# AlgoLab/rs-vgaligner

Measured on AMD Instinct MI355X. Metric: aligned reads/sec (10 kbp ONT vs HLA graph), higher is better.
Workload: dtype int32+f64

## Files before the change

### rs-vgaligner_amd/csrc/vga_poa_row.hpp

```cpp
#pragma once

#include "vga_poa_launch.hpp"
#include "vga_poa_kernels.hpp"

#define T4_NEG (4 * POA_NEG)

template <int B>
__device__ __forceinline__ int t4_sub_byte(int a, int g)
{
    int r;
    if constexpr (B == 0) asm("v_sub_u32_sdwa %0, %1, %2 dst_sel:DWORD dst_unused:UNUSED_PAD src0_sel:DWORD src1_sel:BYTE_0" : "=v"(r) : "v"(a), "v"(g));
    if constexpr (B == 1) asm("v_sub_u32_sdwa %0, %1, %2 dst_sel:DWORD dst_unused:UNUSED_PAD src0_sel:DWORD src1_sel:BYTE_1" : "=v"(r) : "v"(a), "v"(g));
    if constexpr (B == 2) asm("v_sub_u32_sdwa %0, %1, %2 dst_sel:DWORD dst_unused:UNUSED_PAD src0_sel:DWORD src1_sel:BYTE_2" : "=v"(r) : "v"(a), "v"(g));
    if constexpr (B == 3) asm("v_sub_u32_sdwa %0, %1, %2 dst_sel:DWORD dst_unused:UNUSED_PAD src0_sel:DWORD src1_sel:BYTE_3" : "=v"(r) : "v"(a), "v"(g));
    return r;
}
template <int B>
__device__ __forceinline__ void t4_gap_byte(int &dst, int &acc, int t, int c)
{
    if constexpr (B == 0) asm("v_min_u32_sdwa %0, %2, %3 dst_sel:BYTE_0 dst_unused:UNUSED_PRESERVE src0_sel:DWORD src1_sel:DWORD\n\tv_cmp_le_u32 vcc, %3, %2\n\tv_addc_co_u32 %1, vcc, %1, %1, vcc" : "+v"(dst), "+v"(acc) : "v"(t), "s"(c) : "vcc");
    if constexpr (B == 1) asm("v_min_u32_sdwa %0, %2, %3 dst_sel:BYTE_1 dst_unused:UNUSED_PRESERVE src0_sel:DWORD src1_sel:DWORD\n\tv_cmp_le_u32 vcc, %3, %2\n\tv_addc_co_u32 %1, vcc, %1, %1, vcc" : "+v"(dst), "+v"(acc) : "v"(t), "s"(c) : "vcc");
    if constexpr (B == 2) asm("v_min_u32_sdwa %0, %2, %3 dst_sel:BYTE_2 dst_unused:UNUSED_PRESERVE src0_sel:DWORD src1_sel:DWORD\n\tv_cmp_le_u32 vcc, %3, %2\n\tv_addc_co_u32 %1, vcc, %1, %1, vcc" : "+v"(dst), "+v"(acc) : "v"(t), "s"(c) : "vcc");
    if constexpr (B == 3) asm("v_min_u32_sdwa %0, %2, %3 dst_sel:BYTE_3 dst_unused:UNUSED_PRESERVE src0_sel:DWORD src1_sel:DWORD\n\tv_cmp_le_u32 vcc, %3, %2\n\tv_addc_co_u32 %1, vcc, %1, %1, vcc" : "+v"(dst), "+v"(acc) : "v"(t), "s"(c) : "vcc");
}
__device__ __forceinline__ void t4_flag_ne(int &acc, int a, int b)
{
    asm("v_cmp_ne_u32 vcc, %1, %2\n\tv_addc_co_u32 %0, vcc, %0, %0, vcc" : "+v"(acc) : "v"(a), "v"(b) : "vcc");
}
template <int B>
__device__ __forceinline__ void t4_flag_ne_dep(int &dst, int acc, int a, int b)
{
    if constexpr (B == 0) asm("v_cmp_ne_u32 vcc, %2, %3\n\tv_addc_co_u32_sdwa %0, vcc, %1, %1, vcc dst_sel:BYTE_0 dst_unused:UNUSED_PRESERVE src0_sel:DWORD src1_sel:DWORD" : "+v"(dst) : "v"(acc), "v"(a), "v"(b) : "vcc");
    if constexpr (B == 1) asm("v_cmp_ne_u32 vcc, %2, %3\n\tv_addc_co_u32_sdwa %0, vcc, %1, %1, vcc dst_sel:BYTE_1 dst_unused:UNUSED_PRESERVE src0_sel:DWORD src1_sel:DWORD" : "+v"(dst) : "v"(acc), "v"(a), "v"(b) : "vcc");
    if constexpr (B == 2) asm("v_cmp_ne_u32 vcc, %2, %3\n\tv_addc_co_u32_sdwa %0, vcc, %1, %1, vcc dst_sel:BYTE_2 dst_unused:UNUSED_PRESERVE src0_sel:DWORD src1_sel:DWORD" : "+v"(dst) : "v"(acc), "v"(a), "v"(b) : "vcc");
    if constexpr (B == 3) asm("v_cmp_ne_u32 vcc, %2, %3\n\tv_addc_co_u32_sdwa %0, vcc, %1, %1, vcc dst_sel:BYTE_3 dst_unused:UNUSED_PRESERVE src0_sel:DWORD src1_sel:DWORD" : "+v"(dst) : "v"(acc), "v"(a), "v"(b) : "vcc");
}
__device__ __forceinline__ int t4_max3(int a, int b, int c)
{
    int r;
    asm("v_max3_i32 %0, %1, %2, %3" : "=v"(r) : "v"(a), "v"(b), "v"(c));
    return r;
}
__device__ __forceinline__ int t4_shr1_max(int v, int pre)
{
    int r = pre;
    asm("s_nop 1\n\tv_max_i32_dpp %0, %1, %2 wave_shr:1 row_mask:0xf bank_mask:0xf" : "+v"(r) : "v"(v), "v"(pre));
    return r;
}
__device__ __forceinline__ int t4_shr1_mov(int v, int first)
{
    int r = first;
    asm("s_nop 1\n\tv_mov_b32_dpp %0, %1 wave_shr:1 row_mask:0xf bank_mask:0xf" : "+v"(r) : "v"(v));
    return r;
}

template <int B>
__device__ __forceinline__ void t5_min_byte(int &dst, int t, int c)
{
    if constexpr (B == 0) asm("v_min_u32_sdwa %0, %1, %2 dst_sel:BYTE_0 dst_unused:UNUSED_PRESERVE src0_sel:DWORD src1_sel:DWORD" : "+v"(dst) : "v"(t), "s"(c));
    if constexpr (B == 1) asm("v_min_u32_sdwa %0, %1, %2 dst_sel:BYTE_1 dst_unused:UNUSED_PRESERVE src0_sel:DWORD src1_sel:DWORD" : "+v"(dst) : "v"(t), "s"(c));
    if constexpr (B == 2) asm("v_min_u32_sdwa %0, %1, %2 dst_sel:BYTE_2 dst_unused:UNUSED_PRESERVE src0_sel:DWORD src1_sel:DWORD" : "+v"(dst) : "v"(t), "s"(c));
    if constexpr (B == 3) asm("v_min_u32_sdwa %0, %1, %2 dst_sel:BYTE_3 dst_unused:UNUSED_PRESERVE src0_sel:DWORD src1_sel:DWORD" : "+v"(dst) : "v"(t), "s"(c));
}

__device__ __forceinline__ int t5_own(int v)
{
    asm volatile("" : "+v"(v));
    return __builtin_amdgcn_readfirstlane(v);
}
__device__ __forceinline__ uint32_t t5_own(uint32_t v) { return (uint32_t)t5_own((int)v); }
__device__ __forceinline__ uint64_t t5_own(uint64_t v) { return ((uint64_t)t5_own((uint32_t)(v >> 32)) << 32) | t5_own((uint32_t)v); }
template <typename T>
__device__ __forceinline__ T *t5_own(T *p) { return (T *)t5_own((uint64_t)p); }


struct poa_row_view {
    int qlen;
    const char *query;
    const uint4 *ntab;
    const uint32_t *plist, *seqw;
    poa_row *R;
    uint32_t n_nodes, ring_rows;
    int bw, banded, p_match, p_mismatch;
};
__device__ __forceinline__ poa_row_view poa_row_view_of(const poa_prob &pb, const char *queries, const uint4 *node_tab, const uint32_t *seq32,
                                                        const uint32_t *preds, const poa_t5_args &A)
{
    poa_row_view V;
    V.qlen = t5_own((int)pb.qlen);
    V.query = queries + pb.q0;
    V.ntab = node_tab + t5_own(pb.node0);
    V.plist = preds + t5_own(pb.pred0);
    V.seqw = seq32 + t5_own(pb.seq0 >> 2);
    V.R = A.rows + t5_own(pb.row0);
    V.n_nodes = t5_own(pb.n_nodes);
    V.ring_rows = t5_own(pb.ring_rows);
    V.bw = t5_own((int)pb.w);
    V.banded = t5_own(A.P.banded);
    V.p_match = t5_own(A.P.match);
    V.p_mismatch = t5_own(A.P.mismatch);
    return V;
}
struct poa_row_pen {
    int o1, e1, o2, e2, D1, D2;
    uint32_t g_bias, e_probe;
};
template <bool DEF>
__device__ __forceinline__ poa_row_pen poa_row_pen_of(const poa_dev_params &P)
{
    poa_row_pen K;
    K.o1 = DEF ? 4 : t5_own(P.o1); K.e1 = DEF ? 2 : t5_own(P.e1); K.o2 = DEF ? 24 : t5_own(P.o2); K.e2 = DEF ? 1 : t5_own(P.e2);
    K.D1 = 4 * K.o1; K.D2 = 4 * K.o2 + 1;
    K.g_bias = (uint32_t)(4 * K.e1 | (4 * K.e2) << 8) * 0x00010001u;
    K.e_probe = (uint32_t)((128 - K.D1) | (128 - K.D2) << 8) * 0x00010001u;
    return K;
}

__device__ __forceinline__ bool poa_row_state(const poa_t5_args &A, int got, bool first_thread, uint64_t &state_lo)
{
    if (got < 0) {
        if (first_thread) {
            poa_out &O = A.outs[blockIdx.x];
            O.t_end = O.t_begin; O.cells = 0; O.vcells = 0; O.maxw = 0; O.nops = 0;
            O.score = POA_NEG; O.row = 0; O.status = A.cp.n_slots ? POA_ST_POOL : POA_ST_RETRY;
        }
        return false;
    }
    __builtin_amdgcn_fence(__ATOMIC_ACQUIRE, "agent");
    state_lo = (uint64_t)A.cp.state_base + (uint64_t)(uint32_t)got * A.cp.state_size;
    return true;
}

struct poa_chunks {
    uint32_t own_head, own_tail, own_chunks;
    uint64_t dcur;
    uint32_t drem;
};
__device__ __forceinline__ uint32_t poa_chunks_pop(const poa_chunk_pool &cp, const poa_chunks &C)
{
    const uint32_t idx = poa_chunk_pop(cp, blockIdx.x);
    if (idx != POA_NIL) __hip_atomic_store(cp.next + idx, C.own_head, __ATOMIC_RELAXED, __HIP_MEMORY_SCOPE_AGENT);
    return idx;
}
__device__ __forceinline__ void poa_chunks_took(poa_chunks &C, uint32_t idx, uint64_t addr)
{
    C.own_head = idx;
    if (C.own_tail == POA_NIL) C.own_tail = idx;
    C.own_chunks++;
    C.dcur = addr;
    C.drem = (uint32_t)POA_CHUNK;
}
__device__ __forceinline__ uint64_t poa_chunks_bump(poa_chunks &C, uint32_t bytes)
{
    const uint64_t r = C.dcur;
    C.dcur += bytes;
    C.drem -= bytes;
    return r;
}

__device__ __forceinline__ int poa_row_codes(uint16_t *Qn, const char *query, int qlen, int n_hw, int tid, int nt)
{
    int non_acgt = 0;
    for (int t = tid; t < n_hw; t += nt) {
        uint32_t hw = 0;
#pragma unroll
        for (int k = 0; k < 4; k++) {
            const int j = 4 * t + k;
            uint32_t code = 0;
            if (j >= 1 && j <= qlen) {
                const char ch = query[j - 1];
                code = (ch == 'A' || ch == 'C' || ch == 'G' || ch == 'T') ? 1u << (((uint32_t)ch >> 1) & 3u) : 0u;
                non_acgt |= code == 0;
            }
            hw |= code << (4 * k);
        }
        Qn[t] = (uint16_t)hw;
    }
    return non_acgt;
}

struct poa_row_topo {
    uint32_t r;
    bool last;
    bool is_sink;
    uint32_t ps;
    uint32_t gb;
    bool simple;
    bool first;
    int np;
    int remain;
};
__device__ __forceinline__ poa_row_topo poa_row_topo_of(const uint4 nt, uint32_t v, uint32_t tn, const uint32_t *seqw, uint32_t &seq_word,
                                                        uint32_t &seq_word_idx)
{
    const uint32_t nlen = nt.y & 0xFFFFFFu;
    const int np_node = (int)(nt.y >> 24);
    poa_row_topo T;
    T.r = nt.x + tn;
    T.last = tn + 1 == nlen;
    T.is_sink = T.last && (nt.z >> 31) != 0;
    T.ps = nt.w;
    T.gb = 0;
    if (v > 0) {
        const uint32_t bi = T.r - 1;
        if ((bi & 3u) == 0 || (bi >> 2) != seq_word_idx) { seq_word_idx = bi >> 2; seq_word = seqw[seq_word_idx]; }
        T.gb = (seq_word >> (8u * (bi & 3u))) & 0xffu;
    }
    T.simple = T.r > 0 && (tn > 0 || (np_node == 1 && T.ps == T.r - 1));
    T.first = tn == 0 && v > 0;
    T.np = v == 0 ? 0 : (tn == 0 ? np_node : 1);
    T.remain = (int)(nt.z & 0x3fffffffu) + (int)(nlen - 1 - tn);
    return T;
}

__device__ __forceinline__ void poa_row_far_span(const poa_row_view &V, const poa_row_topo &T, int prev_lmax, int prev_rmax, int &mpl, int &mpr)
{
    mpl = INT32_MAX; mpr = 0;
    for (int t = 0; t < T.np; t++) {
        const uint32_t p = T.np == 1 ? T.ps : V.plist[T.ps + t];
        int lm, rm;
        if (p == T.r - 1) { lm = prev_lmax + 1; rm = prev_rmax + 1; }
        else {
            lm = __builtin_amdgcn_readfirstlane(V.R[p].lmax) + 1;
            rm = __builtin_amdgcn_readfirstlane(V.R[p].rmax) + 1;
        }
        mpl = lm < mpl ? lm : mpl;
        mpr = rm > mpr ? rm : mpr;
    }
}
__device__ __forceinline__ void poa_row_band(const poa_row_view &V, const poa_row_topo &T, int mpl, int mpr, int &beg, int &end, int &bal, int &W)
{
    if (!V.banded) { beg = 0; end = V.qlen; }
    else {
        const int diag = V.qlen - T.remain;
        const int lo = mpl < diag ? mpl : diag;
        const int hi = mpr > diag ? mpr : diag;
        beg = lo - V.bw; if (beg < 0) beg = 0;
        end = hi + V.bw; if (end > V.qlen) end = V.qlen;
    }
    bal = beg & ~3;
    W = (end - bal + 1 + 3) & ~3;
}

__device__ __forceinline__ uint32_t poa_row_dir_bytes(int W, int np) { return (uint32_t)W * (np > 1 ? 4u : 1u); }
__device__ __forceinline__ bool poa_row_value_in_chunk(const poa_row_topo &T, const uint4 nt) { return T.r == 0 || (nt.z & 0x40000000u); }
__device__ __forceinline__ uint64_t poa_row_ring_slot(uint64_t ring_base, uint32_t ring_size, uint32_t ring_rows, uint32_t &ring_head)
{
    const uint64_t voff = ring_base + (uint64_t)ring_head * ring_size;
    ring_head = ring_head + 1 == ring_rows ? 0 : ring_head + 1;
    return voff;
}
struct poa_row_counts {
    uint64_t cells, vcells;
    int maxw;
};
__device__ __forceinline__ void poa_row_record(poa_row *R, const poa_row_topo &T, bool first_thread, int beg, int end, int W, uint64_t doff,
                                               uint64_t voff, poa_row_counts &N)
{
    if (T.r > 0) N.cells += (uint64_t)(end - beg + 1);
    if (T.last) N.vcells += (uint64_t)(end - beg + 1);
    N.maxw = W > N.maxw ? W : N.maxw;
    if (first_thread) {
        *(int4 *)&R[T.r].beg = make_int4(beg, end, (int)(uint32_t)doff, (int)(uint32_t)(doff >> 32));
        *(uint2 *)&R[T.r].pred = make_uint2(T.ps, T.first ? (uint32_t)T.np : 0u);
        if (T.last) R[T.r].voff = voff;
    }
}

struct poa_row_base {
    int gsh, ne4t, mm4;
};
__device__ __forceinline__ poa_row_base poa_row_base_of(uint32_t gb, int p_match, int p_mismatch)
{
    const uint32_t gd = gb - (uint32_t)'A';
    const bool acgt = gd < 20u && ((0x80045u >> gd) & 1u);
    const int sc_eq = acgt ? p_match : 0, sc_ne = acgt ? -p_mismatch : 0;
    poa_row_base B;
    B.gsh = (int)((gb >> 1) & 3u);
    B.ne4t = 4 * sc_ne + 1;
    B.mm4 = 4 * (sc_eq - sc_ne);
    return B;
}

struct poa_pred_row {
    const uint8_t *Vq;
    int bp, balq, Wq;
    unsigned pspan;
};
__device__ __forceinline__ poa_pred_row poa_pred_row_of(const poa_row *R, uint32_t p)
{
    poa_pred_row P;
    P.bp = __builtin_amdgcn_readfirstlane(R[p].beg);
    const int ep = __builtin_amdgcn_readfirstlane(R[p].end);
    const uint64_t vq_off = poa_uniform_u64(R[p].voff);
    P.Vq = (const uint8_t *)vq_off;
    P.balq = P.bp & ~3;
    P.Wq = vq_off != 0 ? (ep - P.balq + 1 + 3) & ~3 : 0;
    P.pspan = (unsigned)(ep - P.bp);
    return P;
}
__device__ __forceinline__ void poa_pred_quad(const poa_pred_row &P, int j0, int fill, int4 &hv, uint2 &gg)
{
    const int idx = j0 - P.balq;
    hv = make_int4(fill, fill, fill, fill);
    gg = make_uint2(0u, 0u);
    if (idx >= 0 && idx < P.Wq) {
        hv = *(const int4 *)((const int32_t *)P.Vq + idx);
        gg = *(const uint2 *)(P.Vq + 4ll * P.Wq + 2ll * idx);
    }
}
__device__ __forceinline__ int poa_pred_word(const poa_pred_row &P, int j, int fill)
{
    const int idx = j - P.balq;
    return (idx >= 0 && idx < P.Wq) ? ((const int32_t *)P.Vq)[idx] : fill;
}
__device__ __forceinline__ void poa_stage_quad(const poa_pred_row &P, int j0, int4 &hv, uint2 &gg)
{
    poa_pred_quad(P, j0, T4_NEG + 1, hv, gg);
    const unsigned pspan = P.pspan;
    const bool in0 = (unsigned)(j0 - P.bp) <= pspan, in1 = (unsigned)(j0 + 1 - P.bp) <= pspan, in2 = (unsigned)(j0 + 2 - P.bp) <= pspan,
               in3 = (unsigned)(j0 + 3 - P.bp) <= pspan;
    hv.x = in0 ? hv.x : T4_NEG + 1; hv.y = in1 ? hv.y : T4_NEG + 1; hv.z = in2 ? hv.z : T4_NEG + 1; hv.w = in3 ? hv.w : T4_NEG + 1;
    gg.x = (in0 ? gg.x & 0xffffu : 0u) | (in1 ? gg.x & 0xffff0000u : 0u);
    gg.y = (in2 ? gg.y & 0xffffu : 0u) | (in3 ? gg.y & 0xffff0000u : 0u);
}
__device__ __forceinline__ int poa_stage_word(const poa_pred_row &P, int j)
{
    const int wl = poa_pred_word(P, j, T4_NEG + 1);
    return (unsigned)(j - P.bp) <= P.pspan ? wl : T4_NEG + 1;
}
template <int Q>
struct poa_merged {
    int h[Q][4];
    uint32_t ga[Q], gb[Q];
    int hl;
    bool no_row;
};
template <int Q>
__device__ __forceinline__ poa_merged<Q> poa_stage_merge(const poa_row_view &V, const poa_row_topo &T, int jl, int bal, int W, uint8_t *drow)
{
    poa_merged<Q> M;
    int x1[Q][4], x2[Q][4];
    uint32_t ah[Q], a1[Q], a2[Q];
    uint32_t ahl = 0;
    M.no_row = false;
    M.hl = T4_NEG;
#pragma unroll
    for (int q = 0; q < Q; q++) {
        ah[q] = 0; a1[q] = 0; a2[q] = 0;
#pragma unroll
        for (int k = 0; k < 4; k++) { M.h[q][k] = T4_NEG; x1[q][k] = T4_NEG; x2[q][k] = T4_NEG; }
    }
    for (int t = 0; t < T.np; t++) {
        const poa_pred_row P = poa_pred_row_of(V.R, V.plist[T.ps + t]);
        if (__builtin_expect(P.Vq == nullptr, 0)) M.no_row = true;
#pragma unroll
        for (int q = 0; q < Q; q++) {
            const int j0 = jl + 4 * q;
            int4 hv;
            uint2 gg;
            poa_pred_quad(P, j0, 0, hv, gg);
            const int hj[4] = {hv.x, hv.y, hv.z, hv.w};
            const uint32_t g16[4] = {gg.x & 0xffffu, gg.x >> 16, gg.y & 0xffffu, gg.y >> 16};
#pragma unroll
            for (int k = 0; k < 4; k++) {
// ... 145 lines not shown
```

### rs-vgaligner_amd/csrc/vga_poa_t5.hpp

```cpp
#pragma once

#include "vga_poa_row.hpp"

__device__ __forceinline__ uint64_t t5_uniform64(uint64_t v)
{
    return ((uint64_t)(uint32_t)__builtin_amdgcn_readfirstlane((int)(v >> 32)) << 32) | (uint32_t)__builtin_amdgcn_readfirstlane((int)(uint32_t)v);
}

#define POA_T5_ARGS_OFFSET 40
__device__ __forceinline__ const poa_t5_args *t5_kargs()
{
    uint32_t off = POA_T5_ARGS_OFFSET;
    asm volatile("" : "+s"(off));
    return (const poa_t5_args *)((const char *)__builtin_amdgcn_kernarg_segment_ptr() + off);
}
template <int NT, bool DEF>
__global__ __launch_bounds__(NT) __attribute__((amdgpu_waves_per_eu(5)))
void k_poa_dp_t5(const poa_prob *__restrict__ probs, const char *__restrict__ queries,
                                                       const uint4 *__restrict__ node_tab, const uint32_t *__restrict__ seq32,
                                                       const uint32_t *__restrict__ preds, const poa_t5_args A)
{
    poa_row *rows = A.rows;
    uint8_t *pool_arg = A.pool;
    const uint32_t lds_cols = t5_own(A.lds_cols), hg_cols = t5_own(A.hg_cols), win_mask = t5_own(A.win_mask);
    enum : uint32_t { ST_CHUNKED = 1u, ST_QPLAIN = 2u, ST_FAILED = 4u, ST_PREV_LDS = 8u, ST_PREV_FAR_USE = 16u };
    uint32_t st = (A.cp.n_slots != 0 ? ST_CHUNKED : 0u) | ST_PREV_LDS;
#define chunked ((st & ST_CHUNKED) != 0)
#define failed ((st & ST_FAILED) != 0)
#define q_plain ((st & ST_QPLAIN) != 0)
#define prev_lds ((st & ST_PREV_LDS) != 0)
#define prev_far_use ((st & ST_PREV_FAR_USE) != 0)
    struct { int match, mismatch, o1, e1, o2, e2, banded; } P = {t5_own(A.P.match), t5_own(A.P.mismatch), A.P.o1, A.P.e1, A.P.o2, A.P.e2, t5_own(A.P.banded)};
    constexpr int NW = NT / 64;
    constexpr int STEP = NT * 4;
    extern __shared__ __attribute__((aligned(16))) uint8_t smem[];
    int4 *sX = (int4 *)smem;
    int4 *sRed = sX + 2 * NW;
    int32_t *edgeW = (int32_t *)(sRed + NW);
    int32_t *sSink = edgeW + 4;
    uint64_t *sChunk = (uint64_t *)(sSink + 4);
    constexpr int HDR = (3 * NW + 1 + 1 + 2) * 16;
    int32_t *Hs = (int32_t *)(smem + HDR);
    uint16_t *Gs = (uint16_t *)(smem + HDR + 4ull * hg_cols);
    uint16_t *Qn = (uint16_t *)(smem + HDR + 6ull * hg_cols);
    const int edge_idx = (int)(edgeW - Hs);

    if (threadIdx.x == 0) A.outs[blockIdx.x].t_begin = __builtin_amdgcn_s_memrealtime();
    if (A.prio) __builtin_amdgcn_s_setprio(3);
    const poa_prob pb = probs[blockIdx.x];
    const int tid = threadIdx.x, lane = tid & 63, wv = __builtin_amdgcn_readfirstlane(tid >> 6);
    const int qlen = t5_own((int)pb.qlen);
    const char *query = queries + pb.q0;
    const uint4 *ntab = node_tab + t5_own(pb.node0);
    const uint32_t *plist = preds + t5_own(pb.pred0);
    const uint32_t *seqw = seq32 + t5_own(pb.seq0 >> 2);
    poa_row *R = rows + t5_own(pb.row0);
    const uint32_t n_nodes = t5_own(pb.n_nodes), ring_rows = t5_own(pb.ring_rows);

    uint8_t *pool = pool_arg;
    uint64_t state_lo = 0, state_hi = 0;
    if (chunked) {
        int got = -1;
        if (!(pb.flags & 1u)) {
            if (tid == 0) {
                got = poa_slot_acquire(A.cp.slot_flag, A.cp.n_slots, blockIdx.x);
                sSink[1] = got;
            }
            __syncthreads();
            got = __builtin_amdgcn_readfirstlane(sSink[1]);
        }
        if (got < 0) {
            if (tid == 0) {
                poa_out &O = A.outs[blockIdx.x];
                O.t_end = O.t_begin; O.cells = 0; O.vcells = 0; O.maxw = 0; O.nops = 0;
                O.score = POA_NEG; O.row = 0; O.status = POA_ST_POOL;
            }
            return;
        }
        __builtin_amdgcn_fence(__ATOMIC_ACQUIRE, "agent");
        pool = nullptr;
        state_lo = (uint64_t)A.cp.state_base + (uint64_t)(uint32_t)got * A.cp.state_size;
        state_hi = state_lo + A.cp.state_size;
    }

    const int o1 = DEF ? 4 : P.o1, e1 = DEF ? 2 : P.e1, o2 = DEF ? 24 : P.o2, e2 = DEF ? 1 : P.e2;
    const int C1 = 4 * (o1 + e1), C2 = 4 * (o2 + e2) + 1;
    const int D1 = 4 * o1, D2 = 4 * o2 + 1;
    const uint32_t g_bias = (uint32_t)(4 * e1 | (4 * e2) << 8) * 0x00010001u;
    const uint32_t e_probe = (uint32_t)((128 - D1) | (128 - D2) << 8) * 0x00010001u;
    const int bw = t5_own((int)pb.w);

    uint32_t own_head = POA_NIL, own_chunks = 0;
    auto alloc = [&](uint64_t &cur, uint32_t &rem, uint32_t bytes_asked, int slot) -> uint64_t {
        const uint32_t bytes = (bytes_asked + 15u) & ~15u;
        if (__builtin_expect(bytes > rem, 0)) {
            if (chunked) {
                if (slot == 0 && bytes <= POA_CHUNK) {
                    const poa_t5_args *ka = t5_kargs();
                    if (tid == 0) {
                        const uint32_t idx = poa_chunk_pop(ka->cp, blockIdx.x);
                        if (idx != POA_NIL) __hip_atomic_store(ka->cp.next + idx, own_head, __ATOMIC_RELAXED, __HIP_MEMORY_SCOPE_AGENT);
                        if (own_chunks == 0) sChunk[3] = idx;
                        sChunk[0] = idx;
                    }
                    __syncthreads();
                    const uint32_t idx = (uint32_t)__builtin_amdgcn_readfirstlane((int)(uint32_t)sChunk[0]);
                    __syncthreads();
                    if (idx == POA_NIL) st |= ST_FAILED;
                    else {
                        own_head = idx;
                        own_chunks++;
                        cur = poa_uniform_u64(poa_chunk_addr(ka->cp, idx));
                        rem = (uint32_t)POA_CHUNK;
                    }
                } else
                    st |= ST_FAILED;
                if (failed) return cur;
            } else {
                const uint64_t need = bytes > POA_CHUNK ? ((uint64_t)bytes + POA_CHUNK - 1) & ~(POA_CHUNK - 1) : POA_CHUNK;
                const poa_t5_args *ka = t5_kargs();
                if (tid == 0) sChunk[slot] = atomicAdd(ka->pool_next, (unsigned long long)need);
                __syncthreads();
                const uint64_t b = t5_uniform64(sChunk[slot]);
                __syncthreads();
                if (b + need > ka->pool_size) st |= ST_FAILED;
                cur = b;
                rem = (uint32_t)need;
            }
        }
        const uint64_t r = cur;
        cur += bytes;
        rem -= bytes;
        return r;
    };

    int non_acgt = 0;
    for (int t = tid; t < (int)(lds_cols / 4); t += NT) {
        uint32_t hw = 0;
#pragma unroll
        for (int k = 0; k < 4; k++) {
            const int j = 4 * t + k;
            uint32_t code = 0;
            if (j >= 1 && j <= qlen) {
                const char ch = query[j - 1];
                code = (ch == 'A' || ch == 'C' || ch == 'G' || ch == 'T') ? 1u << (((uint32_t)ch >> 1) & 3u) : 0u;
                non_acgt |= code == 0;
            }
            hw |= code << (4 * k);
        }
        Qn[t] = (uint16_t)hw;
    }
    if (__builtin_amdgcn_readfirstlane(__syncthreads_or(non_acgt)) == 0) st |= ST_QPLAIN;

    uint64_t dcur = 0, vcur = state_lo, wide_scratch = 0, ring_base = 0;
    uint32_t dend = 0, vendp = (uint32_t)(state_hi - state_lo);
    uint32_t ring_head = 0;
    if (win_mask != 0xFFFFFFFFu) wide_scratch = alloc(vcur, vendp, 2u * 6u * lds_cols, 1);
    {
        const uint64_t maxrow = (6ull * (uint64_t)((qlen + 8) & ~3) + 15ull) & ~15ull;
        if (chunked) {
            ring_base = alloc(vcur, vendp, (uint32_t)(maxrow * (uint64_t)ring_rows), 1);
        } else {
            const uint64_t rb = (maxrow * (uint64_t)ring_rows + POA_CHUNK - 1) & ~(POA_CHUNK - 1);
            if (tid == 0) sChunk[2] = atomicAdd(A.pool_next, (unsigned long long)rb);
            __syncthreads();
            const uint64_t b = t5_uniform64(sChunk[2]);
            if (b + rb > A.pool_size || rb >= (1ull << 32)) st |= ST_FAILED;
            ring_base = b;
        }
    }
    if (tid == 0) { sSink[2] = POA_NEG; sSink[3] = 0; }
    int prev_beg = 0, prev_end = -1;
    uint32_t seq_word = 0, seq_word_idx = 0xFFFFFFFFu;

    for (uint32_t v = 0; v < n_nodes && !failed; v++) {
    const uint4 nt = ntab[v];
    const uint32_t nlen = nt.y & 0xFFFFFFu;
    for (uint32_t tn = 0; tn < nlen && !failed; tn++) {
        asm volatile("" : "+s"(st));
        POA_MARK("row_topo");
        const uint32_t r = nt.x + tn;
        const bool last = tn + 1 == nlen;
        const bool is_sink = last && (nt.z >> 31) != 0;
        const uint32_t ps = nt.w;
        uint32_t gb = 0;
        if (v > 0) {
            const uint32_t bi = r - 1;
            if ((bi & 3u) == 0 || (bi >> 2) != seq_word_idx) { seq_word_idx = bi >> 2; seq_word = seqw[seq_word_idx]; }
            gb = (seq_word >> (8u * (bi & 3u))) & 0xffu;
        }
        const bool simple = r > 0 && prev_lds && (tn > 0 || ((nt.y >> 24) == 1u && ps == r - 1));
        const bool writer = wv == (int)(r % (uint32_t)NW);
        POA_MARK("row_prevmax");
        int prev_lmax = 0, prev_rmax = 0;
        if (r > 0) {
            int4 rw = make_int4(INT32_MIN, INT32_MAX, INT32_MIN, 0);
            if (lane < NW) rw = sRed[lane];
            int b = rw.x, t;
            t = poa_dpp<0x111, 0xf>(INT32_MIN, b); b = t > b ? t : b;
            if (NW > 2) { t = poa_dpp<0x112, 0xf>(INT32_MIN, b); b = t > b ? t : b; }
            if (NW > 4) { t = poa_dpp<0x114, 0xf>(INT32_MIN, b); b = t > b ? t : b; }
            if (NW > 8) { t = poa_dpp<0x118, 0xf>(INT32_MIN, b); b = t > b ? t : b; }
            const int rbest = __builtin_amdgcn_readlane(b, NW - 1);
            const uint64_t tie = __builtin_amdgcn_ballot_w64(rw.x == rbest);
            if (__builtin_expect(__builtin_popcountll(tie) == 1, 1)) {
                const int w1 = __builtin_ctzll(tie);
                prev_lmax = __builtin_amdgcn_readlane(rw.y, w1);
                prev_rmax = __builtin_amdgcn_readlane(rw.z, w1);
            } else {
                int lm = rw.x == rbest ? rw.y : INT32_MAX, rm = rw.x == rbest ? rw.z : INT32_MIN;
                t = poa_dpp<0x111, 0xf>(INT32_MAX, lm); lm = t < lm ? t : lm;
                t = poa_dpp<0x111, 0xf>(INT32_MIN, rm); rm = t > rm ? t : rm;
                if (NW > 2) {
                    t = poa_dpp<0x112, 0xf>(INT32_MAX, lm); lm = t < lm ? t : lm;
                    t = poa_dpp<0x112, 0xf>(INT32_MIN, rm); rm = t > rm ? t : rm;
                }
                if (NW > 4) {
                    t = poa_dpp<0x114, 0xf>(INT32_MAX, lm); lm = t < lm ? t : lm;
                    t = poa_dpp<0x114, 0xf>(INT32_MIN, rm); rm = t > rm ? t : rm;
                }
                if (NW > 8) {
                    t = poa_dpp<0x118, 0xf>(INT32_MAX, lm); lm = t < lm ? t : lm;
                    t = poa_dpp<0x118, 0xf>(INT32_MIN, rm); rm = t > rm ? t : rm;
                }
                prev_lmax = __builtin_amdgcn_readlane(lm, NW - 1);
                prev_rmax = __builtin_amdgcn_readlane(rm, NW - 1);
            }
            if (prev_far_use && writer && lane == 0) { R[r - 1].lmax = prev_lmax; R[r - 1].rmax = prev_rmax; }
        }
        POA_MARK("row_setup");
        const int remain = (int)(nt.z & 0x3fffffffu) + (int)(nlen - 1 - tn);
        int beg, end, np, pbeg = prev_beg, pend = prev_end;
        bool first, single, sp_near;
        uint32_t sp = r - 1;
        uint64_t vpo = 0;
        if (__builtin_expect(simple, 1)) {
            first = tn == 0;
            np = 1; single = true; sp_near = true;
            const int mpl = prev_lmax + 1, mpr = prev_rmax + 1;
            if (!P.banded) { beg = 0; end = qlen; }
            else {
                const int diag = qlen - remain;
                const int lo = mpl < diag ? mpl : diag;
                const int hi = mpr > diag ? mpr : diag;
                beg = lo - bw; if (beg < 0) beg = 0;
                end = hi + bw; if (end > qlen) end = qlen;
            }
        } else {
            first = tn == 0 && v > 0;
            np = v == 0 ? 0 : (tn == 0 ? (int)(nt.y >> 24) : 1);
            bool far = r > 0 && !prev_lds;
            if (first) {
                if (np == 1) far |= ps != r - 1;
                else
                    for (int t = 0; t < np; t++) far |= plist[ps + t] != r - 1;
            }
            single = r > 0 && np == 1;
            sp = first ? ps : r - 1;
            sp_near = sp == r - 1 && prev_lds;
            if (far) __syncthreads();
            int mpl, mpr;
            if (r == 0) { mpl = 0; mpr = 0; }
            else if (!first) { mpl = prev_lmax + 1; mpr = prev_rmax + 1; }
            else {
                mpl = INT32_MAX; mpr = 0;
                for (int t = 0; t < np; t++) {
                    const uint32_t p = np == 1 ? ps : plist[ps + t];
                    int lm, rm;
                    if (p == r - 1) { lm = prev_lmax + 1; rm = prev_rmax + 1; }
                    else {
                        lm = __builtin_amdgcn_readfirstlane(R[p].lmax) + 1;
                        rm = __builtin_amdgcn_readfirstlane(R[p].rmax) + 1;
                    }
                    mpl = lm < mpl ? lm : mpl;
                    mpr = rm > mpr ? rm : mpr;
                }
            }
            if (!P.banded) { beg = 0; end = qlen; }
            else {
                const int diag = qlen - remain;
                const int lo = mpl < diag ? mpl : diag;
                const int hi = mpr > diag ? mpr : diag;
                beg = lo - bw; if (beg < 0) beg = 0;
                end = hi + bw; if (end > qlen) end = qlen;
            }
            if (single && !sp_near) {
                pbeg = __builtin_amdgcn_readfirstlane(R[sp].beg);
                pend = __builtin_amdgcn_readfirstlane(R[sp].end);
                vpo = t5_uniform64(R[sp].voff);
            }
        }
        const int bal = beg & ~3;
        const int W = (end - bal + 1 + 3) & ~3;
        const bool wide = (uint32_t)W + 8u > hg_cols;
        const bool keep = last || wide;
        const uint64_t doff = alloc(dcur, dend, (uint32_t)W * (np > 1 ? 4u : 1u), 0);
        uint64_t voff = 0;
        if (last && !failed) {
            if (r == 0 || (nt.z & 0x40000000u)) voff = chunked ? alloc(dcur, dend, 6u * (uint32_t)W, 0) : alloc(vcur, vendp, 6u * (uint32_t)W, 1);
            else {
                voff = ring_base + (uint64_t)ring_head * ((6u * (uint32_t)((qlen + 8) & ~3) + 15u) & ~15u);
                ring_head = ring_head + 1 == ring_rows ? 0 : ring_head + 1;
            }
        } else if (wide) voff = wide_scratch + (r & 1u) * 6ull * lds_cols;
        if (__builtin_expect(failed, 0)) break;
        if (writer && lane == 0) {
            uint32_t *rec = (uint32_t *)(R + r);
            *(uint4 *)rec = make_uint4((uint32_t)beg, (uint32_t)end, (uint32_t)doff, (uint32_t)(doff >> 32));
            *(uint2 *)(rec + 4) = make_uint2((uint32_t)voff, (uint32_t)(voff >> 32));
            *(HIP_vector_type<uint32_t, 3> *)(rec + 8) = HIP_vector_type<uint32_t, 3>(ps, first ? (uint32_t)np : 0u, keep ? 1u : 0u);
        }
        uint8_t *Vrow = pool + voff;
        uint8_t *drow = pool + doff;
        const uint32_t gd = gb - (uint32_t)'A';
        const bool acgt = gd < 20u && ((0x80045u >> gd) & 1u);
        const int sc_eq = acgt ? P.match : 0, sc_ne = acgt ? -P.mismatch : 0;
        const int gsh = (int)((gb >> 1) & 3u);
        const int ne4t = 4 * sc_ne + 1, mm4 = 4 * (sc_eq - sc_ne);
        const bool staged = !simple && r > 0 && !wide && q_plain;
        if (staged) {
            POA_MARK("row_stage");
            if (chunked) {
                bool no_row = false;
                for (int t = 0; t < np; t++) no_row |= t5_uniform64(R[np == 1 ? sp : plist[ps + t]].voff) == 0;
                if (__builtin_expect(no_row, 0)) st |= ST_FAILED;
            }
            for (int c0 = 0; c0 < W; c0 += STEP) {
                const int c = c0 + 4 * tid;
                const int j0 = bal + c;
                if (j0 <= end && np == 1) {
                    const int bp = __builtin_amdgcn_readfirstlane(R[sp].beg), ep = __builtin_amdgcn_readfirstlane(R[sp].end);
                    const uint64_t vq_off = t5_uniform64(R[sp].voff);
                    const uint8_t *Vq = pool + vq_off;
                    const bool vq_ok = !chunked || vq_off != 0;
                    const int balq = bp & ~3;
                    const int Wq = (ep - balq + 1 + 3) & ~3;
                    const int idx = j0 - balq;
                    int4 hv = make_int4(T4_NEG, T4_NEG, T4_NEG, T4_NEG);
                    uint2 gg = make_uint2(0u, 0u);
                    if (idx >= 0 && idx < Wq && vq_ok) {
                        hv = *(const int4 *)((const int32_t *)Vq + idx);
                        gg = *(const uint2 *)(Vq + 4ll * Wq + 2ll * idx);
                    }
                    const unsigned pspan = (unsigned)(ep - bp);
                    const bool in0 = (unsigned)(j0 - bp) <= pspan, in1 = (unsigned)(j0 + 1 - bp) <= pspan, in2 = (unsigned)(j0 + 2 - bp) <= pspan,
                               in3 = (unsigned)(j0 + 3 - bp) <= pspan;
                    hv.x = in0 ? hv.x : T4_NEG; hv.y = in1 ? hv.y : T4_NEG; hv.z = in2 ? hv.z : T4_NEG; hv.w = in3 ? hv.w : T4_NEG;
                    gg.x = (in0 ? gg.x & 0xffffu : 0u) | (in1 ? gg.x & 0xffff0000u : 0u);
                    gg.y = (in2 ? gg.y & 0xffffu : 0u) | (in3 ? gg.y & 0xffff0000u : 0u);
                    *(int4 *)(Hs + (j0 & win_mask)) = hv;
                    *(uint2 *)(Gs + (j0 & win_mask)) = gg;
                    if (c == 0 && bal > 0) {
                        const int wl = (idx >= 1 && idx - 1 < Wq && vq_ok) ? ((const int32_t *)Vq)[idx - 1] : 0;
                        Hs[(bal - 1) & win_mask] = (unsigned)(j0 - 1 - bp) <= pspan ? wl : T4_NEG;
                    }
                } else if (j0 <= end) {
                    int hm[4], x1[4], x2[4], ah[4], a1[4], a2[4];
                    int hl = T4_NEG, ahl = 0;
#pragma unroll
                    for (int k = 0; k < 4; k++) { hm[k] = T4_NEG; x1[k] = T4_NEG; x2[k] = T4_NEG; ah[k] = 0; a1[k] = 0; a2[k] = 0; }
                    for (int t = 0; t < np; t++) {
                        const uint32_t p = np == 1 ? sp : plist[ps + t];
                        const int bp = __builtin_amdgcn_readfirstlane(R[p].beg), ep = __builtin_amdgcn_readfirstlane(R[p].end);
                        const uint64_t vq_off = t5_uniform64(R[p].voff);
                        const uint8_t *Vq = pool + vq_off;
                        const int balq = bp & ~3;
                        const int Wq = (!chunked || vq_off != 0) ? (ep - balq + 1 + 3) & ~3 : 0;
                        const int idx = j0 - balq;
                        int4 hv = make_int4(0, 0, 0, 0);
                        uint2 gg = make_uint2(0u, 0u);
                        if (idx >= 0 && idx < Wq) {
                            hv = *(const int4 *)((const int32_t *)Vq + idx);
                            gg = *(const uint2 *)(Vq + 4ll * Wq + 2ll * idx);
                        }
                        int wl = (idx >= 1 && idx - 1 < Wq) ? ((const int32_t *)Vq)[idx - 1] : 0;
                        const unsigned pspan = (unsigned)(ep - bp);
                        const int hj[4] = {hv.x, hv.y, hv.z, hv.w};
                        const uint32_t g16[4] = {gg.x & 0xffffu, gg.x >> 16, gg.y & 0xffffu, gg.y >> 16};
#pragma unroll
                        for (int k = 0; k < 4; k++) {
                            if ((unsigned)(j0 + k - bp) <= pspan) {
                                const int h = hj[k], c1 = h - (int)(g16[k] & 255u), c2 = h - (int)(g16[k] >> 8);
                                if (h > hm[k]) { hm[k] = h; ah[k] = t; }
                                if (c1 > x1[k]) { x1[k] = c1; a1[k] = t; }
                                if (c2 > x2[k]) { x2[k] = c2; a2[k] = t; }
                            }
                        }
                        if (j0 >= 1 && (unsigned)(j0 - 1 - bp) <= pspan && wl > hl) { hl = wl; ahl = t; }
                    }
                    const int4 hq = make_int4(hm[0], hm[1], hm[2], hm[3]);
                    uint32_t gv[4];
#pragma unroll
                    for (int k = 0; k < 4; k++) gv[k] = (uint32_t)(hm[k] - x1[k]) | ((uint32_t)(hm[k] - x2[k]) << 8);
                    *(int4 *)(Hs + (j0 & win_mask)) = hq;
                    *(uint2 *)(Gs + (j0 & win_mask)) = make_uint2(gv[0] | (gv[1] << 16), gv[2] | (gv[3] << 16));
                    if (c == 0 && bal > 0) Hs[(bal - 1) & win_mask] = hl;
                    if (np > 1) {
                        *(uint32_t *)(drow + (uint64_t)W + c) = (uint32_t)ahl | ((uint32_t)ah[0] << 8) | ((uint32_t)ah[1] << 16) | ((uint32_t)ah[2] << 24);
                        *(uint32_t *)(drow + 2ull * W + c) = (uint32_t)a1[0] | ((uint32_t)a1[1] << 8) | ((uint32_t)a1[2] << 16) | ((uint32_t)a1[3] << 24);
                        *(uint32_t *)(drow + 3ull * W + c) = (uint32_t)a2[0] | ((uint32_t)a2[1] << 8) | ((uint32_t)a2[2] << 16) | ((uint32_t)a2[3] << 24);
                    }
                }
            }
            POA_LDS_BARRIER();
            pbeg = bal > 0 ? bal - 1 : 0;
            pend = bal + W - 1;
        }
        const uint8_t *Vp = pool + vpo;
        const int balp = pbeg & ~3;

        POA_MARK("row_steps");
        enum : uint32_t { F_SINGLE = 1u, F_NEAR = 2u, F_PLAIN = 4u, F_WIDE = 8u, F_KEEP = 16u, F_SINK = 32u, F_MULTI = 64u, F_SRC = 128u };
        const uint32_t rowf = (single ? F_SINGLE : 0u) | (sp_near ? F_NEAR : 0u) | (q_plain ? F_PLAIN : 0u) | (wide ? F_WIDE : 0u) |
                              (keep ? F_KEEP : 0u) | (is_sink ? F_SINK : 0u) | (np > 1 ? F_MULTI : 0u) | (r == 0 ? F_SRC : 0u);
        int best = INT32_MIN, lpos = beg, rpos = beg;
        const bool hot = (simple || staged) && !wide && q_plain;
        const int rlim = end < pend ? end : pend;
        auto run_steps = [&](auto hot_c) __attribute__((always_inline)) {
        constexpr bool HOT = decltype(hot_c)::value;
        int carry1 = POA_IDENT, carry2 = POA_IDENT, left1 = POA_IDENT, left2 = POA_IDENT;
        int next_left = 0;
        int buf = 0;
        for (int c0 = 0; c0 < W; c0 += STEP, buf ^= 1) {
            uint32_t f = HOT ? (rowf & (F_KEEP | F_SINK)) : rowf;
            asm volatile("" : "+s"(f));
            if (HOT) f |= F_SINGLE | F_NEAR | F_PLAIN;
            const int c = c0 + 4 * tid;
            const int j0 = bal + c;
            const bool lane_act = j0 <= end;
            const int jw0 = bal + c0 + 256 * wv, jw1 = jw0 + 255;
            const bool wave_act = jw0 <= end;
            int d_lp = jw0 - beg, d_rp = rlim - jw1, d_lq = (jw0 > beg ? jw0 : beg) - pbeg - 1;
            asm volatile("" : "+s"(d_lp), "+s"(d_rp), "+s"(d_lq));
            const uint32_t e_lp = (uint32_t)d_lp >> 31;
            const uint32_t e_rp = (uint32_t)d_rp >> 31;
            const uint32_t e_lq = (uint32_t)d_lq >> 31;
            const bool lp = e_lp != 0, rp = e_rp != 0, lq = e_lq != 0;
            int htt[4], ht4[4], e1t[4], e2t[4], pmeta[4];
            int agg1 = POA_IDENT, agg2 = POA_IDENT, alast1 = POA_IDENT, alast2 = POA_IDENT;
#pragma unroll
            for (int k = 0; k < 4; k++) { htt[k] = T4_NEG + 2; ht4[k] = T4_NEG; e1t[k] = T4_NEG + 1; e2t[k] = T4_NEG; pmeta[k] = 0; }
            uint32_t qn = 0u;
            if (wave_act) qn = (uint32_t)Qn[j0 >> 2];
            const bool fastw = HOT ? wave_act
                                   : (f & (F_SINGLE | F_PLAIN)) == (F_SINGLE | F_PLAIN) && wave_act && (!lq || (f & F_NEAR)) && (!rp || ((f & F_NEAR) && end <= pend + 1));
            const int base1 = 4 * e1 * j0, base2 = 4 * e2 * j0;
        if constexpr (HOT) POA_MARK("hot_p1_fast"); else POA_MARK("p1_fast");
            if (__builtin_expect(fastw, 1)) {
                int4 hv;
                uint2 gg;
                int hprev;
                if constexpr (HOT) {
                    hv = *(const int4 *)(Hs + (j0 & win_mask));
                    gg = *(const uint2 *)(Gs + (j0 & win_mask));
                    int left0;
                    if (wv == 0 && c0 > 0) left0 = next_left;
                    else left0 = Hs[(jw0 > 0 ? jw0 - 1 : 0) & (int)win_mask];
                    if (wv == 0 && c0 + STEP < W) next_left = Hs[(jw0 + STEP - 1) & (int)win_mask];
                    hprev = t4_shr1_mov(hv.w, left0);
                } else if (__builtin_expect((f & F_NEAR) != 0, 1)) {
                    hv = *(const int4 *)(Hs + (j0 & win_mask));
                    gg = *(const uint2 *)(Gs + (j0 & win_mask));
                    if (tid == NT - 1) edgeW[buf] = hv.w;
                    {
                        const bool edge = tid == 0 && c0 > 0;
                        int w = Hs[edge ? edge_idx + (buf ^ 1) : ((j0 > 0 ? j0 - 1 : 0) & win_mask)];
                        asm volatile("" : "+v"(w));
                        hprev = w;
                    }
                } else {
                    const int Wp = (pend - balp + 1 + 3) & ~3;
                    const int idx = j0 - balp;
                    hv = *(const int4 *)((const int32_t *)Vp + idx);
                    gg = *(const uint2 *)(Vp + 4ll * Wp + 2ll * idx);
                    hprev = ((const int32_t *)Vp)[idx > 0 ? idx - 1 : 0];
                    asm volatile("" : "+v"(hv.x), "+v"(hv.y), "+v"(hv.z), "+v"(hv.w), "+v"(gg.x), "+v"(gg.y), "+v"(hprev));
                }
                auto phase1 = [&](auto edge_c) {
                    constexpr bool EDGE = decltype(edge_c)::value;
                    int hj[4] = {hv.x, hv.y, hv.z, hv.w};
                    int ga = (int)gg.x, gbb = (int)gg.y;
                    if constexpr (EDGE) {
                        if (rp) {
#pragma unroll
                            for (int k = 0; k < 4; k++) hj[k] = j0 + k > pend ? T4_NEG : hj[k];
                            ga = j0 > pend ? 0 : (j0 + 1 > pend ? (ga & 0xffff) : ga);
                            gbb = j0 + 2 > pend ? 0 : (j0 + 3 > pend ? (gbb & 0xffff) : gbb);
                        }
                        if (lq) {
#pragma unroll
                            for (int k = 0; k < 4; k++) hj[k] = j0 + k < pbeg ? T4_NEG : hj[k];
                            ga = j0 + 1 < pbeg ? 0 : (j0 < pbeg ? (int)((uint32_t)ga & 0xffff0000u) : ga);
                            gbb = j0 + 3 < pbeg ? 0 : (j0 + 2 < pbeg ? (int)((uint32_t)gbb & 0xffff0000u) : gbb);
                        }
                    }
                    const uint32_t eqb = qn >> gsh;
                    int hp = hprev;
                    if constexpr (EDGE && HOT) {
                        if (rp) hp = j0 - 1 > pend ? T4_NEG : hp;
                    }
#pragma unroll
                    for (int k = 0; k < 4; k++) {
                        const int g = k < 2 ? ga : gbb;
                        const int ev1 = (k & 1) ? t4_sub_byte<2>(hj[k], g) : t4_sub_byte<0>(hj[k], g);
                        const int ev2 = (k & 1) ? t4_sub_byte<3>(hj[k], g) : t4_sub_byte<1>(hj[k], g);
                        int m = (int)__umul24(__builtin_amdgcn_ubfe(eqb, 4u * k, 1u), (uint32_t)mm4) + (hp + ne4t);
                        if constexpr (EDGE) {
                            if (lq) m = j0 + k - 1 < pbeg ? T4_NEG + 2 : m;
                        }
                        const int h = t4_max3(m, ev1, ev2);
                        htt[k] = h;
                        ht4[k] = h & ~3;
                        e1t[k] = ev1;
                        e2t[k] = ev2;
                        hp = hj[k];
                    }
                    if constexpr (EDGE) {
                        if (lp) {
#pragma unroll
                            for (int k = 0; k < 4; k++) ht4[k] = j0 + k < beg ? POA_IDENT : ht4[k];
                        }
                    }
                    const int r11 = ht4[1] + 4 * e1, r12 = ht4[2] + 8 * e1, r13 = ht4[3] + 12 * e1;
                    const int r21 = ht4[1] + 4 * e2, r22 = ht4[2] + 8 * e2, r23 = ht4[3] + 12 * e2;
                    const int a1 = t4_max3(ht4[0], r11, r12), a2 = t4_max3(ht4[0], r21, r22);
                    agg1 = (a1 > r13 ? a1 : r13) + base1;
                    agg2 = (a2 > r23 ? a2 : r23) + base2;
                    alast1 = r13 + base1;
                    alast2 = r23 + base2;
                };
                if (__builtin_expect((e_lp | e_rp | e_lq) != 0, 0)) phase1(std::true_type{});
                else phase1(std::false_type{});
        if constexpr (HOT) POA_MARK("hot_p1_lean"); else POA_MARK("p1_lean");
            } else if (wave_act && (f & F_SINGLE)) {
                int pbeg_ = pbeg, pend_ = pend, beg_ = beg, end_ = end, balp_ = balp, gsh_ = gsh;
                asm volatile("" : "+s"(pbeg_), "+s"(pend_), "+s"(beg_), "+s"(end_), "+s"(balp_), "+s"(gsh_));
                const int pbeg = pbeg_, pend = pend_, beg = beg_, end = end_, balp = balp_, gsh = gsh_;
                const unsigned span = (unsigned)(end - beg), pspan = (unsigned)(pend - pbeg);
                int hj[4], wm0;
                uint32_t g16[4];
                if (f & F_NEAR) {
                    const int4 hv = *(const int4 *)(Hs + (j0 & win_mask));
                    const uint2 gg = *(const uint2 *)(Gs + (j0 & win_mask));
                    hj[0] = hv.x; hj[1] = hv.y; hj[2] = hv.z; hj[3] = hv.w;
                    g16[0] = gg.x & 0xffffu; g16[1] = gg.x >> 16; g16[2] = gg.y & 0xffffu; g16[3] = gg.y >> 16;
                    if (tid == NT - 1) edgeW[buf] = hj[3];
                    const bool edge = tid == 0 && c0 > 0;
                    int w = Hs[edge ? edge_idx + (buf ^ 1) : ((j0 > 0 ? j0 - 1 : 0) & win_mask)];
                    asm volatile("" : "+v"(w));
                    wm0 = w;
                } else {
                    const int idx = j0 - balp;
                    const int Wp = (pend - balp + 1 + 3) & ~3;
                    int4 hv = make_int4(0, 0, 0, 0);
                    uint2 gg = make_uint2(0u, 0u);
                    if (idx >= 0 && idx < Wp) {
                        hv = *(const int4 *)((const int32_t *)Vp + idx);
                        gg = *(const uint2 *)(Vp + 4ll * Wp + 2ll * idx);
                    }
                    wm0 = (idx >= 1 && idx - 1 < Wp) ? ((const int32_t *)Vp)[idx - 1] : 0;
                    asm volatile("" : "+v"(hv.x), "+v"(hv.y), "+v"(hv.z), "+v"(hv.w), "+v"(gg.x), "+v"(gg.y), "+v"(wm0));
                    hj[0] = hv.x; hj[1] = hv.y; hj[2] = hv.z; hj[3] = hv.w;
                    g16[0] = gg.x & 0xffffu; g16[1] = gg.x >> 16; g16[2] = gg.y & 0xffffu; g16[3] = gg.y >> 16;
                }
                bool inprev = j0 >= 1 && (unsigned)(j0 - 1 - pbeg) <= pspan;
#pragma unroll
                for (int k = 0; k < 4; k++) {
                    const int j = j0 + k;
                    const bool inj = (unsigned)(j - pbeg) <= pspan;
                    const bool actk = (unsigned)(j - beg) <= span;
                    const int qc = (int)((qn >> (4 * k)) & 15u);
                    const int s = ((qc >> gsh) & 1) ? sc_eq : (qc == 0 ? 0 : sc_ne);
                    const int wm = k == 0 ? wm0 : hj[k - 1];
                    const int m = inprev ? wm + 4 * s + 1 : T4_NEG + 2;
                    const int ev1 = inj ? hj[k] - (int)(g16[k] & 255u) : T4_NEG + 1;
                    const int ev2 = inj ? hj[k] - (int)(g16[k] >> 8) : T4_NEG;
                    const int h = t4_max3(m, ev1, ev2);
                    htt[k] = h;
                    ht4[k] = h & ~3;
                    e1t[k] = ev1;
                    e2t[k] = ev2;
                    const int a1 = actk ? ht4[k] + 4 * e1 * j : POA_IDENT, a2 = actk ? ht4[k] + 4 * e2 * j : POA_IDENT;
                    agg1 = a1 > agg1 ? a1 : agg1;
                    agg2 = a2 > agg2 ? a2 : agg2;
                    if (k == 3) { alast1 = a1; alast2 = a2; }
                    inprev = inj;
                }
        if constexpr (HOT) POA_MARK("hot_p1_general"); else POA_MARK("p1_general");
            } else if (wave_act) {
                int beg_ = beg, end_ = end, gsh_ = gsh;
                asm volatile("" : "+s"(beg_), "+s"(end_), "+s"(gsh_));
                const int beg = beg_, end = end_, gsh = gsh_;
                const unsigned span = (unsigned)(end - beg);
                if (f & F_SRC) {
#pragma unroll
                    for (int k = 0; k < 4; k++) { ht4[k] = (j0 + k == 0) ? 0 : T4_NEG; htt[k] = ht4[k] + 2; }
                } else if (lane_act) {
                    int m[4], ev1[4], ev2[4];
#pragma unroll
                    for (int k = 0; k < 4; k++) { m[k] = T4_NEG + 2; ev1[k] = T4_NEG + 1; ev2[k] = T4_NEG; }
                    for (int t = 0; t < np; t++) {
                        const uint32_t p = plist[ps + t];
                        int hj[4], wm0 = 0;
                        uint32_t g16[4];
                        int bp, ep;
                        if (p == r - 1 && prev_lds) {
                            bp = prev_beg; ep = prev_end;
                            const int4 hv = *(const int4 *)(Hs + (j0 & win_mask));
                            const uint2 gg = *(const uint2 *)(Gs + (j0 & win_mask));
                            hj[0] = hv.x; hj[1] = hv.y; hj[2] = hv.z; hj[3] = hv.w;
                            g16[0] = gg.x & 0xffffu; g16[1] = gg.x >> 16; g16[2] = gg.y & 0xffffu; g16[3] = gg.y >> 16;
                            if (tid == NT - 1) edgeW[buf] = hj[3];
                            const bool edge = tid == 0 && c0 > 0;
                            int w = Hs[edge ? edge_idx + (buf ^ 1) : ((j0 > 0 ? j0 - 1 : 0) & win_mask)];
                            asm volatile("" : "+v"(w));
                            wm0 = w;
                        } else {
                            bp = __builtin_amdgcn_readfirstlane(R[p].beg);
                            ep = __builtin_amdgcn_readfirstlane(R[p].end);
                            const uint64_t vo = R[p].voff;
                            const uint64_t vos = ((uint64_t)(uint32_t)__builtin_amdgcn_readfirstlane((int)(vo >> 32)) << 32) |
                                                 (uint32_t)__builtin_amdgcn_readfirstlane((int)(uint32_t)vo);
                            const uint8_t *Vq = pool + vos;
                            const int balq = bp & ~3;
                            const int Wq = (ep - balq + 1 + 3) & ~3;
                            const int idx = j0 - balq;
                            int4 hv = make_int4(0, 0, 0, 0);
                            uint2 gg = make_uint2(0u, 0u);
                            if (idx >= 0 && idx < Wq) {
                                hv = *(const int4 *)((const int32_t *)Vq + idx);
                                gg = *(const uint2 *)(Vq + 4ll * Wq + 2ll * idx);
                            }
                            wm0 = (idx >= 1 && idx - 1 < Wq) ? ((const int32_t *)Vq)[idx - 1] : 0;
                            asm volatile("" : "+v"(hv.x), "+v"(hv.y), "+v"(hv.z), "+v"(hv.w), "+v"(gg.x), "+v"(gg.y), "+v"(wm0));
                            hj[0] = hv.x; hj[1] = hv.y; hj[2] = hv.z; hj[3] = hv.w;
// ... 310 lines not shown
```

Baseline: 10640.

## Add fast interior path for staging predecessor rows with one or two predecessors

Hoists the predecessor row metadata (beg, end, voff) out of the per-chunk staging loop and precomputes per-lane base pointers. For wave-sized chunks that lie entirely inside the predecessor's valid span, the H and gap bytes are copied without bounds masking. A new fully unrolled merge path handles two-predecessor rows using SDWA byte compare and subtract helpers, recording predecessor-choice bits into the direction row. This removes per-column range checks and repeated uniform loads, at the cost of more inline-asm code, higher register pressure and a more complex edge-case split.

New measurement: 10730, median of 6. No clear change (+0.8%).

```diff
diff --git a/rs-vgaligner_amd/csrc/vga_poa_row.hpp b/rs-vgaligner_amd/csrc/vga_poa_row.hpp
--- a/rs-vgaligner_amd/csrc/vga_poa_row.hpp
+++ b/rs-vgaligner_amd/csrc/vga_poa_row.hpp
@@ -61,6 +61,22 @@
     if constexpr (B == 1) asm("v_min_u32_sdwa %0, %1, %2 dst_sel:BYTE_1 dst_unused:UNUSED_PRESERVE src0_sel:DWORD src1_sel:DWORD" : "+v"(dst) : "v"(t), "s"(c));
     if constexpr (B == 2) asm("v_min_u32_sdwa %0, %1, %2 dst_sel:BYTE_2 dst_unused:UNUSED_PRESERVE src0_sel:DWORD src1_sel:DWORD" : "+v"(dst) : "v"(t), "s"(c));
     if constexpr (B == 3) asm("v_min_u32_sdwa %0, %1, %2 dst_sel:BYTE_3 dst_unused:UNUSED_PRESERVE src0_sel:DWORD src1_sel:DWORD" : "+v"(dst) : "v"(t), "s"(c));
+}
+template <int B>
+__device__ __forceinline__ void t5_gt_byte(int &dst, int a, int b)
+{
+    if constexpr (B == 0) asm("v_cmp_gt_i32 vcc, %1, %2\n\tv_cndmask_b32_sdwa %0, 0, 1, vcc dst_sel:BYTE_0 dst_unused:UNUSED_PAD src0_sel:DWORD src1_sel:DWORD" : "=v"(dst) : "v"(a), "v"(b) : "vcc");
+    if constexpr (B == 1) asm("v_cmp_gt_i32 vcc, %1, %2\n\tv_cndmask_b32_sdwa %0, 0, 1, vcc dst_sel:BYTE_1 dst_unused:UNUSED_PRESERVE src0_sel:DWORD src1_sel:DWORD" : "+v"(dst) : "v"(a), "v"(b) : "vcc");
+    if constexpr (B == 2) asm("v_cmp_gt_i32 vcc, %1, %2\n\tv_cndmask_b32_sdwa %0, 0, 1, vcc dst_sel:BYTE_2 dst_unused:UNUSED_PRESERVE src0_sel:DWORD src1_sel:DWORD" : "+v"(dst) : "v"(a), "v"(b) : "vcc");
+    if constexpr (B == 3) asm("v_cmp_gt_i32 vcc, %1, %2\n\tv_cndmask_b32_sdwa %0, 0, 1, vcc dst_sel:BYTE_3 dst_unused:UNUSED_PRESERVE src0_sel:DWORD src1_sel:DWORD" : "+v"(dst) : "v"(a), "v"(b) : "vcc");
+}
+template <int B>
+__device__ __forceinline__ void t5_diff_byte(int &dst, int a, int b)
+{
+    if constexpr (B == 0) asm("v_sub_u32_sdwa %0, %1, %2 dst_sel:BYTE_0 dst_unused:UNUSED_PAD src0_sel:DWORD src1_sel:DWORD" : "=v"(dst) : "v"(a), "v"(b));
+    if constexpr (B == 1) asm("v_sub_u32_sdwa %0, %1, %2 dst_sel:BYTE_1 dst_unused:UNUSED_PRESERVE src0_sel:DWORD src1_sel:DWORD" : "+v"(dst) : "v"(a), "v"(b));
+    if constexpr (B == 2) asm("v_sub_u32_sdwa %0, %1, %2 dst_sel:BYTE_2 dst_unused:UNUSED_PRESERVE src0_sel:DWORD src1_sel:DWORD" : "+v"(dst) : "v"(a), "v"(b));
+    if constexpr (B == 3) asm("v_sub_u32_sdwa %0, %1, %2 dst_sel:BYTE_3 dst_unused:UNUSED_PRESERVE src0_sel:DWORD src1_sel:DWORD" : "+v"(dst) : "v"(a), "v"(b));
 }
 
 __device__ __forceinline__ int t5_own(int v)
diff --git a/rs-vgaligner_amd/csrc/vga_poa_t5.hpp b/rs-vgaligner_amd/csrc/vga_poa_t5.hpp
--- a/rs-vgaligner_amd/csrc/vga_poa_t5.hpp
+++ b/rs-vgaligner_amd/csrc/vga_poa_t5.hpp
@@ -320,17 +320,92 @@
         const bool staged = !simple && r > 0 && !wide && q_plain;
         if (staged) {
             POA_MARK("row_stage");
-            if (chunked) {
+            int vbpa = 0, vepa = -1, lo1 = INT32_MAX, hi = INT32_MIN;
+            uint64_t vvoa = 0;
+            const uint8_t *pha = nullptr, *pga = nullptr, *phb = nullptr, *pgb = nullptr;
+            if (np <= 2) {
+                const uint32_t pa = np == 1 ? sp : plist[ps];
+                vbpa = R[pa].beg; vepa = R[pa].end; vvoa = R[pa].voff;
+                asm volatile("" : "+v"(vbpa), "+v"(vepa), "+v"(vvoa));
+                int vlo = vbpa, vhi = vepa;
+                bool no_row = vvoa == 0;
+                {
+                    const int balq = vbpa & ~3;
+                    pha = pool + vvoa + 4ll * (bal + 4 * tid - balq);
+                    pga = pool + vvoa + 4ll * ((vepa - balq + 1 + 3) & ~3) + 2ll * (bal + 4 * tid - balq);
+                }
+                if (np == 2) {
+                    const uint32_t pq = plist[ps + 1];
+                    int vbpb = R[pq].beg, vepb = R[pq].end;
+                    uint64_t vvob = R[pq].voff;
+                    asm volatile("" : "+v"(vbpb), "+v"(vepb), "+v"(vvob));
+                    vlo = vbpb > vlo ? vbpb : vlo;
+                    vhi = vepb < vhi ? vepb : vhi;
+                    no_row |= vvob == 0;
+                    const int balq = vbpb & ~3;
+                    phb = pool + vvob + 4ll * (bal + 4 * tid - balq);
+                    pgb = pool + vvob + 4ll * ((vepb - balq + 1 + 3) & ~3) + 2ll * (bal + 4 * tid - balq);
+                }
+                lo1 = __builtin_amdgcn_readfirstlane(vlo) + 1; if (lo1 < 1) lo1 = 1;
+                hi = __builtin_amdgcn_readfirstlane(vhi); if (hi > end) hi = end;
+                if (__builtin_expect(chunked && __builtin_amdgcn_readfirstlane((int)no_row) != 0, 0)) { st |= ST_FAILED; hi = INT32_MIN; }
+            } else if (chunked) {
                 bool no_row = false;
-                for (int t = 0; t < np; t++) no_row |= t5_uniform64(R[np == 1 ? sp : plist[ps + t]].voff) == 0;
+                for (int t = 0; t < np; t++) no_row |= t5_uniform64(R[plist[ps + t]].voff) == 0;
                 if (__builtin_expect(no_row, 0)) st |= ST_FAILED;
             }
             for (int c0 = 0; c0 < W; c0 += STEP) {
                 const int c = c0 + 4 * tid;
                 const int j0 = bal + c;
-                if (j0 <= end && np == 1) {
-                    const int bp = __builtin_amdgcn_readfirstlane(R[sp].beg), ep = __builtin_amdgcn_readfirstlane(R[sp].end);
-                    const uint64_t vq_off = t5_uniform64(R[sp].voff);
+                const int jw0 = bal + c0 + 256 * wv;
+                const bool interior = jw0 >= lo1 && jw0 + 255 <= hi;
+                if (interior && np == 1) {
+                    const int4 hv = *(const int4 *)(pha + 4ll * c0);
+                    const uint2 gg = *(const uint2 *)(pga + 2ll * c0);
+                    *(int4 *)(Hs + (j0 & win_mask)) = hv;
+                    *(uint2 *)(Gs + (j0 & win_mask)) = gg;
+                    if (c == 0) Hs[(bal - 1) & win_mask] = *(const int32_t *)(pha - 4);
+                } else if (interior) {
+                    int4 hv = *(const int4 *)(pha + 4ll * c0);
+                    uint2 gg = *(const uint2 *)(pga + 2ll * c0);
+                    int hm[4] = {hv.x, hv.y, hv.z, hv.w}, x1[4], x2[4];
+                    int hl = *(const int32_t *)(pha + 4ll * c0 - 4);
+                    x1[0] = t4_sub_byte<0>(hm[0], (int)gg.x); x2[0] = t4_sub_byte<1>(hm[0], (int)gg.x);
+                    x1[1] = t4_sub_byte<2>(hm[1], (int)gg.x); x2[1] = t4_sub_byte<3>(hm[1], (int)gg.x);
+                    x1[2] = t4_sub_byte<0>(hm[2], (int)gg.y); x2[2] = t4_sub_byte<1>(hm[2], (int)gg.y);
+                    x1[3] = t4_sub_byte<2>(hm[3], (int)gg.y); x2[3] = t4_sub_byte<3>(hm[3], (int)gg.y);
+                    asm volatile("" : "+v"(x1[0]), "+v"(x1[1]), "+v"(x1[2]), "+v"(x1[3]), "+v"(x2[0]), "+v"(x2[1]), "+v"(x2[2]), "+v"(x2[3]));
+                    hv = *(const int4 *)(phb + 4ll * c0);
+                    gg = *(const uint2 *)(pgb + 2ll * c0);
+                    const int wl = *(const int32_t *)(phb + 4ll * c0 - 4);
+                    const int hb[4] = {hv.x, hv.y, hv.z, hv.w};
+                    int y1[4], y2[4];
+                    y1[0] = t4_sub_byte<0>(hb[0], (int)gg.x); y2[0] = t4_sub_byte<1>(hb[0], (int)gg.x);
+                    y1[1] = t4_sub_byte<2>(hb[1], (int)gg.x); y2[1] = t4_sub_byte<3>(hb[1], (int)gg.x);
+                    y1[2] = t4_sub_byte<0>(hb[2], (int)gg.y); y2[2] = t4_sub_byte<1>(hb[2], (int)gg.y);
+                    y1[3] = t4_sub_byte<2>(hb[3], (int)gg.y); y2[3] = t4_sub_byte<3>(hb[3], (int)gg.y);
+                    int pm, p1, p2, ga, gbb;
+                    t5_gt_byte<0>(pm, wl, hl); t5_gt_byte<1>(pm, hb[0], hm[0]); t5_gt_byte<2>(pm, hb[1], hm[1]); t5_gt_byte<3>(pm, hb[2], hm[2]);
+                    t5_gt_byte<0>(p1, y1[0], x1[0]); t5_gt_byte<1>(p1, y1[1], x1[1]); t5_gt_byte<2>(p1, y1[2], x1[2]); t5_gt_byte<3>(p1, y1[3], x1[3]);
+                    t5_gt_byte<0>(p2, y2[0], x2[0]); t5_gt_byte<1>(p2, y2[1], x2[1]); t5_gt_byte<2>(p2, y2[2], x2[2]); t5_gt_byte<3>(p2, y2[3], x2[3]);
+                    hl = wl > hl ? wl : hl;
+#pragma unroll
+                    for (int k = 0; k < 4; k++) {
+                        hm[k] = hb[k] > hm[k] ? hb[k] : hm[k];
+                        x1[k] = y1[k] > x1[k] ? y1[k] : x1[k];
+                        x2[k] = y2[k] > x2[k] ? y2[k] : x2[k];
+                    }
+                    t5_diff_byte<0>(ga, hm[0], x1[0]); t5_diff_byte<1>(ga, hm[0], x2[0]); t5_diff_byte<2>(ga, hm[1], x1[1]); t5_diff_byte<3>(ga, hm[1], x2[1]);
+                    t5_diff_byte<0>(gbb, hm[2], x1[2]); t5_diff_byte<1>(gbb, hm[2], x2[2]); t5_diff_byte<2>(gbb, hm[3], x1[3]); t5_diff_byte<3>(gbb, hm[3], x2[3]);
+                    *(int4 *)(Hs + (j0 & win_mask)) = make_int4(hm[0], hm[1], hm[2], hm[3]);
+                    *(uint2 *)(Gs + (j0 & win_mask)) = make_uint2((uint32_t)ga, (uint32_t)gbb);
+                    if (c == 0) Hs[(bal - 1) & win_mask] = hl;
+                    *(uint32_t *)(drow + (uint64_t)W + c) = (uint32_t)pm;
+                    *(uint32_t *)(drow + 2ull * W + c) = (uint32_t)p1;
+                    *(uint32_t *)(drow + 3ull * W + c) = (uint32_t)p2;
+                } else if (j0 <= end && np == 1) {
+                    const int bp = __builtin_amdgcn_readfirstlane(vbpa), ep = __builtin_amdgcn_readfirstlane(vepa);
+                    const uint64_t vq_off = t5_uniform64(vvoa);
                     const uint8_t *Vq = pool + vq_off;
                     const bool vq_ok = !chunked || vq_off != 0;
                     const int balq = bp & ~3;
```
